# Wendison/FCL-taco2

Hardware: AMD Instinct MI355X
Metric: mel-frames/sec (FCL-taco2-S forward, batch=32, 80-mel) (higher is better)
Workload: dtype f32 via bf16x3-split MFMA operands, fp32 accumulate (max-abs 8e-6 on mel vs the reference; FCL_PRECISION=0 = exact fp32 MFMA)

## Files before the change

fcl-taco2_amd/csrc/capi.hip:

```cpp
#include <stdarg.h>
#include <stdlib.h>
#include <string.h>

#include <map>
#include <mutex>
#include <utility>
#include <vector>

#include "fcl_common.h"

namespace fcl {

static thread_local char g_err[512] = "";
static thread_local int g_gemm_mode = FCL_GEMM_F32;

void set_error(const char* fmt, ...) {
    va_list ap;
    va_start(ap, fmt);
    vsnprintf(g_err, sizeof(g_err), fmt, ap);
    va_end(ap);
}

int check_hip(hipError_t e, const char* what) {
    static const int sync_debug = getenv("FCL_SYNC_DEBUG") ? atoi(getenv("FCL_SYNC_DEBUG")) : 0;
// ... 505 lines not shown
        if (rc) return rc;
        GemmArgs f = {};
        f.term[0] = GemmTerm{io->att_c, w->wf_att, C, C, C, 0};
        if (planes) { f.term[0].Ap = io->att_c_p; f.term[0].Wp = w->wf_att_p; f.term[0].lda_p = f.term[0].ldw_p = ldc; }
        f.nterms = 1; f.M = N; f.N = O; f.Y = ws.F0; f.ldy = O;
        rc = launch_gemm(f, s);
        if (rc) return rc;
    }
    const float keep_scale = 1.0f / (1.0f - w->prenet_dropout);
    const int drop_mode = (w->prenet_dropout > 0.f) ? io->dropout_mode : FCL_DROP_NONE;
    {
        static const int tile_on = tunable("DEC_TILE", 0), tile_min = tunable("DEC_TILE_MIN_ROWS", 1024);
        if (tile_on && planes && w->stream && decoder_tile_shape_ok(w) && N >= tile_min && io->lmax <= 64 && !io->teacher_ys && !io->tap_prenet && !io->tap_lstm0 &&
            !io->tap_lstm1 && drop_mode != FCL_DROP_MASK && gemm_mode() != FCL_GEMM_BF16) {
            hipLaunchKernelGGL(zero_kernel, dim3(512), dim3(256), 0, s, ws.c0, (long long)((ws.c1 - ws.c0) + (size_t)N * U));
            FCL_HIP(hipGetLastError());
            return launch_decoder_tile(w, io, ws.G0, ws.F0, ws.c0, ws.c1, drop_mode, 0, nullptr, nullptr, s);
        }
    }
    const bool tile_ok = planes && w->stream && decoder_tile_shape_ok(w) && io->lmax <= 64 && !io->teacher_ys && !io->tap_prenet && !io->tap_lstm0 && !io->tap_lstm1 &&
                         drop_mode != FCL_DROP_MASK && gemm_mode() != FCL_GEMM_BF16;
    const int tail_from = (tile_ok && io->tail_from > 0 && io->tail_from < io->lmax) ? io->tail_from : 0;
    int cur = 0;
    for (int t = 0; t <= io->lmax; ++t) {
        const bool hand_over = tail_from > 0 && t == tail_from;
        const int n = (t < io->lmax && !hand_over) ? io->live_rows_host[t] : 0;
        const int n_prev = t > 0 ? io->live_rows_host[t - 1] : 0;
        const uint8_t* keep0 = drop_mode == FCL_DROP_MASK && t < io->lmax ? io->prenet_keep + ((size_t)(t * 2 + 0) * N) * P : nullptr;
        const uint8_t* keep1 = drop_mode == FCL_DROP_MASK && t < io->lmax ? io->prenet_keep + ((size_t)(t * 2 + 1) * N) * P : nullptr;
        const unsigned seed0 = io->seed * 2654435761u + (unsigned)(t * 2 + 0), seed1 = seed0 + 1;
        const float* teacher_in = (io->teacher_ys && t > 0) ? io->teacher_ys + (size_t)(t - 1) * O : nullptr;
        FeatPrenetArgs fp = {};
        fp.M_feat = n_prev; fp.M_pre = n; fp.U = U; fp.O = O; fp.P = P;
        fp.h1 = t > 0 ? ws.h1[cur] : nullptr; fp.wf_h = w->wf_h; fp.F0 = ws.F0;
        fp.before = io->before; fp.frame_off = io->frame_off; fp.t_prev = t - 1; fp.t_cur = t;
        fp.teacher_in = teacher_in; fp.teacher_ld = io->lmax * O;
        if (t < io->lmax && !hand_over) { fp.w0 = w->prenet_w0; fp.b0 = w->prenet_b0; fp.w1 = w->prenet_w1; fp.b1 = w->prenet_b1; }
        fp.wf_hi = w->wf_h_hi; fp.wf_lo = w->wf_h_lo; fp.w0_hi = w->prenet_w0_hi; fp.w0_lo = w->prenet_w0_lo;
        fp.w1_hi = w->prenet_w1_hi; fp.w1_lo = w->prenet_w1_lo;
        fp.wf_ff = w->wf_h_ff; fp.w0_ff = w->prenet_w0_ff; fp.w1_ff = w->prenet_w1_ff;
        fp.drop_mode = drop_mode; fp.keep0 = keep0; fp.keep1 = keep1; fp.keep_scale = keep_scale; fp.drop_p = w->prenet_dropout;
        fp.seed0 = seed0; fp.seed1 = seed1; fp.seed_dev = io->seed_dev; fp.pre_out = ws.pre_b; fp.tap_prenet = io->tap_prenet;
        fp.live = io->live_rows; fp.status = io->status; fp.out_act = w->out_act;
        if (planes) {
            fp.before_p = io->before_p;
            if (!small_step(n)) { fp.pre_out_p = ws.pre_p; fp.pre_out = nullptr; }
        }
        int rc = launch_feat_prenet(fp, s);
        if (rc) return rc;
        if (hand_over) return launch_decoder_tile(w, io, ws.G0, ws.F0, ws.c0, ws.c1, drop_mode, t, ws.h0[cur], ws.h1[cur], s);
        if (t == io->lmax) break;
        LstmStepArgs l0 = {};
        const bool big = planes && !small_step(n);
        const bool next_big = planes && t + 1 < io->lmax && !small_step(io->live_rows_host[t + 1]);
        l0.term[0] = GemmTerm{ws.pre_b, w->w0_pre, P, P, P, 0, w->w0_pre_hi, w->w0_pre_lo};
        l0.term[1] = GemmTerm{ws.h0[cur], w->w0_hh, U, U, U, 0, w->w0_hh_hi, w->w0_hh_lo};
        if (big) {
            l0.term[0].Ap = ws.pre_p; l0.term[0].Wp = w->w0_pre_p; l0.term[0].lda_p = l0.term[0].ldw_p = ldp;
            l0.term[1].Ap = ws.h0_p[cur]; l0.term[1].Wp = w->w0_hh_p; l0.term[1].lda_p = l0.term[1].ldw_p = ldu;
            l0.h_out_p = ws.h0_p[cur ^ 1]; l0.ld_hp = ldu;
        }
        l0.term[0].Wff = w->w0_pre_ff; l0.term[1].Wff = w->w0_hh_ff;
        l0.nterms = t == 0 ? 1 : 2; l0.M = n; l0.U = U; l0.G = ws.G0; l0.g_row_mul = 1; l0.g_row_add = 0;
        l0.m_dev = io->live_rows ? io->live_rows + t : nullptr;
        l0.rank1_w = w->w0_pos; l0.dur = io->dur; l0.step = t;
        l0.h_in = t == 0 ? nullptr : ws.h0[cur]; l0.h_out = ws.h0[cur ^ 1]; l0.c = ws.c0; l0.zoneout = w->zoneout_rate;
        if (io->tap_lstm0) { l0.out2 = io->tap_lstm0; l0.out2_row_base = io->frame_off; l0.out2_row_add = t; l0.ld2 = U; }
        rc = launch_lstm_step(l0, s);
        if (rc) return rc;
        LstmStepArgs l1 = {};
        l1.term[0] = GemmTerm{ws.h0[cur ^ 1], w->w1_ih, U, U, U, 0, w->w1_ih_hi, w->w1_ih_lo};
        l1.term[1] = GemmTerm{ws.h1[cur], w->w1_hh, U, U, U, 0, w->w1_hh_hi, w->w1_hh_lo};
        if (big) {
            l1.term[0].Ap = ws.h0_p[cur ^ 1]; l1.term[0].Wp = w->w1_ih_p; l1.term[0].lda_p = l1.term[0].ldw_p = ldu;
            l1.term[1].Ap = ws.h1_p[cur]; l1.term[1].Wp = w->w1_hh_p; l1.term[1].lda_p = l1.term[1].ldw_p = ldu;
            if (next_big) { l1.h_out_p = ws.h1_p[cur ^ 1]; l1.ld_hp = ldu; }
        }
        l1.term[0].Wff = w->w1_ih_ff; l1.term[1].Wff = w->w1_hh_ff;
        l1.nterms = t == 0 ? 1 : 2; l1.M = n; l1.U = U; l1.bias = w->b1; l1.step = t;
        l1.m_dev = l0.m_dev;
        l1.h_in = t == 0 ? nullptr : ws.h1[cur]; l1.h_out = ws.h1[cur ^ 1]; l1.c = ws.c1; l1.zoneout = w->zoneout_rate;
        if (io->tap_lstm1) { l1.out2 = io->tap_lstm1; l1.out2_row_base = io->frame_off; l1.out2_row_add = t; l1.ld2 = U; }
        rc = launch_lstm_step(l1, s);
        if (rc) return rc;
        cur ^= 1;
    }
    return 0;
}

}
```

fcl-taco2_amd/csrc/decoder_step.hip:

```cpp
#include "fcl_common.h"
#include "lstm_epilogue.h"

namespace fcl {


template <int NT>
__device__ __forceinline__ void rowtile_mma(const float* A_l, int lda_l, const float* const (&wrow)[NT], int K, int r16, int kq,
                                            f32x4 (&out)[NT], int rot = 0) {
    f32x4 acc0[NT], acc1[NT];
#pragma unroll
    for (int t = 0; t < NT; ++t) acc0[t] = acc1[t] = (f32x4){0.f, 0.f, 0.f, 0.f};
    const float* ap = A_l + r16 * lda_l + kq * 4;
    const float* wp[NT];
#pragma unroll
    for (int t = 0; t < NT; ++t) wp[t] = wrow[t] + kq * 4;
    const int nfull = K >> 6;
    f32x4 bn[NT][4];
    int cc = nfull > 0 ? rot % nfull : 0;
    if (nfull > 0) {
#pragma unroll
        for (int t = 0; t < NT; ++t)
#pragma unroll
            for (int i = 0; i < 4; ++i) bn[t][i] = *reinterpret_cast<const f32x4*>(wp[t] + (cc << 6) + i * 16);
    }
// ... 555 lines not shown

#ifdef FCL_FP_TS
constexpr int kFpTsWorkgroups = 1024;
__device__ long long g_fp_ts[kFpTsWorkgroups * 8 * 8];
struct FpStamps {
    long long t[8] = {0, 0, 0, 0, 0, 0, 0, 0};
    template <int I>
    __device__ __forceinline__ void at(bool drain = false) {
        __builtin_amdgcn_sched_barrier(0);
        if (drain) asm volatile("s_waitcnt vmcnt(0)" ::: "memory");
        asm volatile("s_memtime %0\n\ts_waitcnt lgkmcnt(0)" : "=s"(t[I])::"memory");
        __builtin_amdgcn_sched_barrier(0);
    }
    __device__ __forceinline__ void flush() {
        at<7>();
        if ((threadIdx.x & 63) == 0 && blockIdx.x < kFpTsWorkgroups) {
#pragma unroll
            for (int i = 0; i < 8; ++i) g_fp_ts[(blockIdx.x * 8 + (threadIdx.x >> 6)) * 8 + i] = t[i];
        }
    }
};
#define FP_STAMP(ts, i, ...) ts.at<i>(__VA_ARGS__)
#define FP_STAMP_FLUSH(ts) ts.flush()
#else
struct FpStamps {};
#define FP_STAMP(ts, i, ...)
#define FP_STAMP_FLUSH(ts)
#endif

template <class Ops, int DROP, int RT>
__global__ __launch_bounds__(512) void feat_prenet_split_kernel(const FeatPrenetArgs a) {
    typedef typename Ops::Tile Tile;
    constexpr int SU = 8, SO = 3, SP = 8, U = 256, OP = 96, P = 256;
    const int M_feat = a.M_feat, M_pre = a.M_pre;
    int Ms_feat, Ms_pre;
    if (!feat_prenet_rows(a, 16 * RT, Ms_feat, Ms_pre)) return;
    [[maybe_unused]] FpStamps ts;
    FP_STAMP(ts, 0);
    constexpr int ldU = U + Ops::PAD, ldO = OP + Ops::PAD, ldP = P + Ops::PAD, ROWS = 16 * RT;
    static_assert(ldU == ldP, "the layer-1 operand tile re-uses the h1 tile's LDS");
    auto* lds = Ops::dynamic_lds();
    const Tile A1 = Tile::carve(lds, ROWS * ldU);
    const Tile A2 = Tile::carve(lds, ROWS * ldO);
    const Tile A3 = A1;
    const int O = a.O;
    const int m0 = blockIdx.x * ROWS;
    const int lane = threadIdx.x & 63, wave = __builtin_amdgcn_readfirstlane(threadIdx.x >> 6);
    const int r16 = lane & 15, kq = lane >> 4;
    const int arow = lane & 15, cq = lane >> 4;
    const bool has_feat = a.h1 != nullptr, has_pre = a.w0 != nullptr && m0 < M_pre;
    const bool feat_wave = has_feat && wave * 16 < O;
    const size_t lane8 = (size_t)lane * 8;
    auto frag = [&](const typename Ops::W w, int tile, int ns) { return w.at((size_t)tile * ns * 512, lane8); };
    const int t0 = wave, t1 = wave + 8;
    const int c1 = wave * 2;

    constexpr int HV = RT * 2;
    f32x4 hreg[HV];
    if (has_feat) {
#pragma unroll
        for (int j = 0; j < HV; ++j) {
            const int i = threadIdx.x + j * 512, r = i >> 6, c = (i & 63) * 4;
            hreg[j] = *reinterpret_cast<const f32x4*>(a.h1 + (size_t)min(m0 + r, M_feat - 1) * U + c);
        }
    }
    asm volatile("s_barrier" ::: "memory");
    typename Ops::template Frag<1, SU> ff;
    typename Ops::template Frag<2, SO> f0;
    typename Ops::template Frag<2, SP> f1;
    const int fnc = wave * 16 + cq * 4;
    f32x4 f0v[RT];
    int fo[RT];
    if (feat_wave) {
        const typename Ops::W w[1] = {frag(Ops::wf(a), wave, SU)};
        ff.load(w);
    }
#pragma unroll
    for (int q = 0; q < RT; ++q) {
        f0v[q] = (f32x4){0.f, 0.f, 0.f, 0.f};
        fo[q] = 0;
        if (feat_wave && fnc < O) {
            const int mc = min(m0 + q * 16 + arow, M_feat - 1);
            f0v[q] = *reinterpret_cast<const f32x4*>(a.F0 + (size_t)mc * O + fnc);
            fo[q] = a.frame_off[mc];
        }
    }
    unsigned int seed0 = 0, seed1 = 0;
    const unsigned int thr16 = (unsigned int)(a.drop_p * 65536.0f);
    if (DROP == 2) {
        const unsigned int sbump = a.seed_dev ? *a.seed_dev * 0x9E3779B9u : 0u;
        seed0 = hash_u32(a.seed0 + sbump);
        seed1 = hash_u32(a.seed1 + sbump);
    }
    f32x4 pb0[2], pb1[2];
    unsigned int k0[RT][2], k1[RT][2];
#pragma unroll
    for (int tt = 0; tt < 2; ++tt) pb0[tt] = (f32x4){0.f, 0.f, 0.f, 0.f};
    if (has_feat) asm volatile("s_barrier" ::: "memory");
    if (has_pre) {
        const typename Ops::W w[2] = {frag(Ops::w0(a), t0, SO), frag(Ops::w0(a), t1, SO)};
        f0.load(w);
#pragma unroll
        for (int tt = 0; tt < 2; ++tt) {
            const int nc = (tt ? t1 : t0) * 16 + cq * 4;
            pb0[tt] = *reinterpret_cast<const f32x4*>(a.b0 + nc);
            if (DROP == 1) {
#pragma unroll
                for (int q = 0; q < RT; ++q) k0[q][tt] = *reinterpret_cast<const unsigned int*>(a.keep0 + (size_t)min(m0 + q * 16 + arow, M_pre - 1) * P + nc);
            }
        }
    }
    Ops::zero(A2, ROWS * ldO);
    if (has_feat) {
#pragma unroll
        for (int j = 0; j < HV; ++j) {
            const int i = threadIdx.x + j * 512, r = i >> 6, c = (i & 63) * 4;
// ... 2 lines not shown
    }
    FP_STAMP(ts, 1);
#pragma unroll
    for (int tt = 0; tt < 2; ++tt) pb1[tt] = (f32x4){0.f, 0.f, 0.f, 0.f};
    auto request_l1 = [&]() {
        if (has_pre) {
            typename Ops::W w[2];
#pragma unroll
            for (int tt = 0; tt < 2; ++tt) w[tt] = frag(Ops::w1(a), c1 + tt, SP);
            f1.load(w);
#pragma unroll
            for (int tt = 0; tt < 2; ++tt) {
                const int nc = (c1 + tt) * 16 + cq * 4;
                pb1[tt] = *reinterpret_cast<const f32x4*>(a.b1 + nc);
                if (DROP == 1) {
#pragma unroll
                    for (int q = 0; q < RT; ++q) k1[q][tt] = *reinterpret_cast<const unsigned int*>(a.keep1 + (size_t)min(m0 + q * 16 + arow, M_pre - 1) * P + nc);
                }
            }
        }
    };
    lds_barrier();
    FP_STAMP(ts, 2);
    if (feat_wave) {
#pragma unroll
        for (int q = 0; q < RT; ++q) {
            f32x4 accv[1];
            ff.mma_t(A1.at(q * 16 * ldU), ldU, r16, kq, accv);
            const int row = q * 16 + arow, m = m0 + row;
            if (fnc < O) {
                f32x4 v = (f32x4){0.f, 0.f, 0.f, 0.f};
                if (m < Ms_feat) {
                    v = accv[0] + f0v[q];
                    const long long fr = (long long)fo[q] + a.t_prev;
                    *reinterpret_cast<f32x4*>(a.before + (size_t)fr * O + fnc) = v;
                    if constexpr (Ops::kPlanes) {
                        if (a.before_p) {
                            uint2 h, l;
                            split4(v, h, l);
                            p32_store4(a.before_p, (O + 31) >> 5, fr, fnc, h, l);
                        }
                    }
                    if (a.out_act) {
#pragma unroll
                        for (int r = 0; r < 4; ++r) v[r] = act_apply(v[r], a.out_act);
                    }
                }
                Ops::store4(A2, row, ldO, fnc, v);
            }
        }
    }
    if (Ops::kPlanes && has_feat && a.before_p && (O & 31)) {
        const int padc = 32 - (O & 31);
        for (int i = threadIdx.x; i < ROWS * padc; i += 512) {
            const int m = m0 + i / padc;
            if (m < Ms_feat) store_p32(a.before_p, (O + 31) >> 5, a.frame_off[m] + a.t_prev, O + i % padc, 0.f);
        }
    }
    FP_STAMP(ts, 3);
    if (!has_pre) {
        FP_STAMP_FLUSH(ts);
        return;
    }
    request_l1();
    lds_barrier();
    if constexpr (Ops::kPlanes) {
        if (a.teacher_in) {
#pragma unroll
            for (int q = 0; q < RT; ++q) load_rowtile_split(A2.h + q * 16 * ldO, A2.l + q * 16 * ldO, ldO, a.teacher_in, a.teacher_ld, O, m0 + q * 16, M_pre);
            lds_barrier();
        }
    }
    FP_STAMP(ts, 4);
#pragma unroll
    for (int q = 0; q < RT; ++q) {
        f32x4 accv[2];
        f0.mma_t(A2.at(q * 16 * ldO), ldO, r16, kq, accv);
        const int row = q * 16 + arow, m = m0 + row;
#pragma unroll
// ... 14 lines not shown
        f32x4 accv[2];
        f1.mma_t(A3.at(q * 16 * ldP), ldP, r16, kq, accv);
        const int m = m0 + q * 16 + arow;
        if (m >= Ms_pre) continue;
#pragma unroll
        for (int tt = 0; tt < 2; ++tt) {
            const int nc = (c1 + tt) * 16 + cq * 4;
            f32x4 v = accv[tt] + pb1[tt];
#pragma unroll
            for (int r = 0; r < 4; ++r) v[r] = fmaxf(v[r], 0.f);
            v = drop4<DROP>(v, DROP == 1 ? k1[q][tt] : 0u, (unsigned int)m * (unsigned int)P + (unsigned int)nc, seed1, thr16, a.keep_scale);
            if (a.pre_out) *reinterpret_cast<f32x4*>(a.pre_out + (size_t)m * P + nc) = v;
            if constexpr (Ops::kPlanes) {
                if (a.pre_out_p) {
                    uint2 h, l;
                    split4(v, h, l);
                    p32_store4(a.pre_out_p, SP, m, nc, h, l);
                }
            }
            if (a.tap_prenet) *reinterpret_cast<f32x4*>(a.tap_prenet + (size_t)(a.frame_off[m] + a.t_cur) * P + nc) = v;
        }
    }
    FP_STAMP_FLUSH(ts);
}

__device__ __forceinline__ void glds16_unseen(const void* g, const void* l) {
    typedef const __attribute__((address_space(3))) void* lds_t;
    const unsigned dst = __builtin_amdgcn_readfirstlane((unsigned)(uintptr_t)(lds_t)l);
    unsigned keep;
    asm volatile("s_mov_b32 %0, m0\n\ts_mov_b32 m0, %2\n\ts_nop 0\n\tglobal_load_lds_dwordx4 %1, off\n\ts_mov_b32 m0, %0" : "=&s"(keep) : "v"(g), "s"(dst) : "memory");
}

template <int DROP, bool FEAT, bool PRE>
__device__ __forceinline__ void feat_prenet_walk(const FeatPrenetArgs& a, const int ntw, const int Ms_feat, const int Ms_pre) {
    typedef OpsX3 Ops;
    typedef Ops::Tile Tile;
    constexpr int SU = 8, SO = 3, SP = 8, U = 256, OP = 96, P = 256;
    constexpr int ldU = U + Ops::PAD, ldO = OP + Ops::PAD, ldP = P + Ops::PAD;
    constexpr int BUF = 2 * 16 * (ldU + ldO);
    static_assert(ldU == ldP, "the layer-1 operand tile re-uses the h1 tile's LDS");
    const int M_feat = a.M_feat, M_pre = a.M_pre;
    [[maybe_unused]] FpStamps ts;
    FP_STAMP(ts, 0);
    const int O = a.O;
    const int lane = threadIdx.x & 63, wave = __builtin_amdgcn_readfirstlane(threadIdx.x >> 6);
    const int r16 = lane & 15, kq = lane >> 4;
// ... 51 lines not shown
                const int i = threadIdx.x + j * 512, r = i >> 6, c = (i & 63) * 4;
                Ops::store4(A1.at(buf * BUF), r, ldU, c, hrow[j]);
            }
        }
    };

    if (feat_wave) {
        const Ops::W w = frag(Ops::wf(a), wave, SU);
#pragma unroll
        for (int st = 0; st < SU; ++st) {
            glds16_unseen(w.hi + st * 512, WF + st * 512);
            glds16_unseen(w.lo + st * 512, WF + (SU + st) * 512);
        }
    }
    request_rows(mbeg);
    asm volatile("s_barrier" ::: "memory");
    request_feat(mbeg);
    request_keep(k0, a.keep0, mbeg, t0, t1);
    request_keep(k1, a.keep1, mbeg, c1, c1 + 1);
    Ops::Frag<2, SO> f0;
    Ops::Frag<2, SP> f1;
    unsigned int seed0 = 0, seed1 = 0;
    const unsigned int thr16 = (unsigned int)(a.drop_p * 65536.0f);
    if (DROP == 2) {
        const unsigned int sbump = a.seed_dev ? *a.seed_dev * 0x9E3779B9u : 0u;
        seed0 = hash_u32(a.seed0 + sbump);
        seed1 = hash_u32(a.seed1 + sbump);
    }
    f32x4 bias = (f32x4){0.f, 0.f, 0.f, 0.f};
    const bool bias_thread = pre_any && threadIdx.x < 2 * (P / 4);
    if (pre_any) {
        if (bias_thread) bias = *reinterpret_cast<const f32x4*>((threadIdx.x < P / 4 ? a.b0 : a.b1 - P) + threadIdx.x * 4);
        const Ops::W w0[2] = {frag(Ops::w0(a), t0, SO), frag(Ops::w0(a), t1, SO)};
        f0.load(w0);
        const Ops::W w1[2] = {frag(Ops::w1(a), c1, SP), frag(Ops::w1(a), c1 + 1, SP)};
        f1.load(w1);
    }
    store_rows(0);
    if (bias_thread) *reinterpret_cast<f32x4*>(BL + threadIdx.x * 4) = bias;
    FP_STAMP(ts, 1);

    auto tile = [&](const int q) {
        const int buf = q & 1, m0 = mbeg + q * 16;
        const Tile T1 = A1.at(buf * BUF), T2 = A2.at(buf * BUF);
        const bool has_pre = pre_any && m0 < M_pre;
        lds_barrier();
        if (q == 0) FP_STAMP(ts, 2);
        if (feat_wave) {
            f32x4 acc = (f32x4){0.f, 0.f, 0.f, 0.f};
            const u16* ah = T1.h + r16 * ldU + kq * 8;
            const u16* al = T1.l + r16 * ldU + kq * 8;
            const u16* wf = WF + lane8;
#pragma unroll
            for (int st = 0; st < SU; ++st) {
                const s16x8 a_hi = *reinterpret_cast<const s16x8*>(ah + st * 32), a_lo = *reinterpret_cast<const s16x8*>(al + st * 32);
                const s16x8 w_hi = *reinterpret_cast<const s16x8*>(wf + st * 512), w_lo = *reinterpret_cast<const s16x8*>(wf + (SU + st) * 512);
                acc = __builtin_amdgcn_mfma_f32_16x16x32_bf16(w_hi, a_lo, acc, 0, 0, 0);
                acc = __builtin_amdgcn_mfma_f32_16x16x32_bf16(w_lo, a_hi, acc, 0, 0, 0);
                acc = __builtin_amdgcn_mfma_f32_16x16x32_bf16(w_hi, a_hi, acc, 0, 0, 0);
            }
            const int m = m0 + arow;
            if (fnc < O) {
                f32x4 v = (f32x4){0.f, 0.f, 0.f, 0.f};
                if (m < Ms_feat) {
                    v = acc + f0v;
                    const long long fr = (long long)fo + a.t_prev;
                    *reinterpret_cast<f32x4*>(a.before + (size_t)fr * O + fnc) = v;
                    if (a.before_p) {
                        uint2 h, l;
                        split4(v, h, l);
                        p32_store4(a.before_p, (O + 31) >> 5, fr, fnc, h, l);
                        if (pad_lane) p32_store4(a.before_p, (O + 31) >> 5, fr, padc, make_uint2(0u, 0u), make_uint2(0u, 0u));
                    }
                    if (a.out_act) {
#pragma unroll
                        for (int r = 0; r < 4; ++r) v[r] = act_apply(v[r], a.out_act);
                    }
                }
                Ops::store4(T2, arow, ldO, fnc, v);
            }
        }
        request_rows(m0 + 16);
        request_feat(m0 + 16);
        if (q == 0) FP_STAMP(ts, 3);
        f32x4 out1[2];
        if (has_pre) {
            lds_barrier();
            if (a.teacher_in) {
                load_rowtile_split(T2.h, T2.l, ldO, a.teacher_in, a.teacher_ld, O, m0, M_pre);
                lds_barrier();
            }
            if (q == 0) FP_STAMP(ts, 4);
            {
                f32x4 accv[2];
                f0.mma_t(T2, ldO, r16, kq, accv);
                const int m = m0 + arow;
#pragma unroll
                for (int tt = 0; tt < 2; ++tt) {
                    const int nc = (tt ? t1 : t0) * 16 + cq * 4;
                    f32x4 v = accv[tt] + *reinterpret_cast<const f32x4*>(BL + nc);
#pragma unroll
                    for (int r = 0; r < 4; ++r) v[r] = fmaxf(v[r], 0.f);
                    v = drop4<DROP>(v, DROP == 1 ? k0[tt] : 0u, (unsigned int)m * (unsigned int)P + (unsigned int)nc, seed0, thr16, a.keep_scale);
                    Ops::store4(T1, arow, ldP, nc, v);
                }
            }
            request_keep(k0, a.keep0, m0 + 16, t0, t1);
            lds_barrier();
            if (q == 0) {
                FP_STAMP(ts, 5);
                FP_STAMP(ts, 6, true);
            }
            f1.mma_t(T1, ldP, r16, kq, out1);
        }
        store_rows(buf ^ 1);
        asm volatile("" : "+v"(f0v), "+v"(fo), "+v"(k0[0]), "+v"(k0[1]));
        if (has_pre) {
            const int m = m0 + arow;
            if (m < Ms_pre) {
#pragma unroll
                for (int tt = 0; tt < 2; ++tt) {
                    const int nc = (c1 + tt) * 16 + cq * 4;
                    f32x4 v = out1[tt] + *reinterpret_cast<const f32x4*>(BL + P + nc);
#pragma unroll
                    for (int r = 0; r < 4; ++r) v[r] = fmaxf(v[r], 0.f);
                    v = drop4<DROP>(v, DROP == 1 ? k1[tt] : 0u, (unsigned int)m * (unsigned int)P + (unsigned int)nc, seed1, thr16, a.keep_scale);
                    if (a.pre_out) *reinterpret_cast<f32x4*>(a.pre_out + (size_t)m * P + nc) = v;
                    if (a.pre_out_p) {
                        uint2 h, l;
                        split4(v, h, l);
                        p32_store4(a.pre_out_p, SP, m, nc, h, l);
                    }
                    if (a.tap_prenet) *reinterpret_cast<f32x4*>(a.tap_prenet + (size_t)(a.frame_off[m] + a.t_cur) * P + nc) = v;
                }
            }
            request_keep(k1, a.keep1, m0 + 16, c1, c1 + 1);
        }
    };
    tile(0);
#pragma unroll 1
    for (int q = 1; q < nt; ++q) tile(q);
    FP_STAMP_FLUSH(ts);
}

template <int DROP>
__global__ __launch_bounds__(512) void feat_prenet_walk_kernel(const FeatPrenetArgs a, const int ntw) {
    int Ms_feat, Ms_pre;
    if (!feat_prenet_rows(a, 16 * ntw, Ms_feat, Ms_pre)) return;
    const bool pre = a.w0 != nullptr && (int)blockIdx.x * 16 * ntw < a.M_pre;
    if (a.h1 != nullptr) {
        if (pre) feat_prenet_walk<DROP, true, true>(a, ntw, Ms_feat, Ms_pre);
        else feat_prenet_walk<DROP, true, false>(a, ntw, Ms_feat, Ms_pre);
    } else if (pre) {
        feat_prenet_walk<DROP, false, true>(a, ntw, Ms_feat, Ms_pre);
    }
}

__device__ __forceinline__ void gates_to_cell(const LstmStepArgs& a, int g, int lane, const f32x4& acc, bool units_in_lane, int m, int u, bool valid, int Ms,
                                              const CellIn& ci) {
    __shared__ float g_l[4][16][17];
    const int lo = lane & 15, hi = lane >> 4;
#pragma unroll
    for (int i = 0; i < 4; ++i) {
        if (units_in_lane) g_l[g][lo][hi * 4 + i] = acc[i];
        else g_l[g][hi * 4 + i][lo] = acc[i];
    }
    __syncthreads();
    if (!valid || m >= Ms) return;
    const int row = threadIdx.x >> 4, uc = threadIdx.x & 15;
    const float pre[4] = {g_l[0][row][uc], g_l[1][row][uc], g_l[2][row][uc], g_l[3][row][uc]};
    cell_finish(a, m, u, pre, ci);
}

constexpr int kSmallStepsAtEntry = 4;

template <class Ops, int NT>
__device__ __forceinline__ f32x4 small_walk(const LstmStepArgs& a, typename Ops::Tile A, int ldk, int m0, int M, int g, int u0, int lane) {
// ... 193 lines not shown
        }
    }
    fprintf(stderr, "fp_ts %s rows %d workgroups %d: cycles since entry, mean (max):", form, rows, wgs);
    static const char* const name[8] = {"", "rows->LDS", "barrier0", "phase1", "barrier1", "phase2+barrier2", "all landed", "exit"};
    for (int i = 1; i < 8; ++i) fprintf(stderr, "  %s %.0f (%.0f)", name[i], cnt[i] ? sum[i] / cnt[i] : 0.0, mx[i]);
    fprintf(stderr, "\n");
    void* p = nullptr;
    if (hipGetSymbolAddress(&p, HIP_SYMBOL(g_fp_ts)) == hipSuccess) (void)hipMemset(p, 0, sizeof(h));
}
#else
static void print_fp_stamps(const char*, int, int) {}
#endif

static int launch_feat_prenet_walk(const FeatPrenetArgs& a, int rows, int ntw, hipStream_t s) {
    const size_t lds_w = sizeof(u16) * ((size_t)((a.O + 15) / 16) * 2 * 8 * 512 + 2 * 2 * 16 * ((256 + OpsX3::PAD) + (96 + OpsX3::PAD))) + 2 * 256 * sizeof(float);
    static const void* const fn[3] = {reinterpret_cast<const void*>(feat_prenet_walk_kernel<0>), reinterpret_cast<const void*>(feat_prenet_walk_kernel<1>),
                                      reinterpret_cast<const void*>(feat_prenet_walk_kernel<2>)};
    const int tiles = (rows + 15) / 16, wgs = (tiles + ntw - 1) / ntw;
    const int rc = launch_fp_drop(fn, a.drop_mode, dim3(wgs, 1), lds_w, a, s, ntw);
    if (!rc) print_fp_stamps("walk", rows, wgs);
    return rc;
}

template <class Ops, int RT>
static int launch_feat_prenet_split(const FeatPrenetArgs& a, int rows, hipStream_t s) {
    constexpr size_t lds_s = (size_t)Ops::LDS_BYTES * 16 * RT * ((256 + Ops::PAD) + (96 + Ops::PAD));
    static const void* const fn[3] = {reinterpret_cast<const void*>(feat_prenet_split_kernel<Ops, 0, RT>), reinterpret_cast<const void*>(feat_prenet_split_kernel<Ops, 1, RT>),
                                      reinterpret_cast<const void*>(feat_prenet_split_kernel<Ops, 2, RT>)};
    const int wgs = (rows + 16 * RT - 1) / (16 * RT);
    const int rc = launch_fp_drop(fn, a.drop_mode, dim3(wgs, 1), lds_s, a, s);
    if (!rc && Ops::kPlanes) print_fp_stamps(RT == 2 ? "split RT=2" : "split RT=1", rows, wgs);
    return rc;
}

int launch_feat_prenet(const FeatPrenetArgs& a, hipStream_t s) {
    const int rows = a.h1 ? a.M_feat : a.M_pre;
    if (rows <= 0) return 0;
    FCL_REQUIRE(!(a.U & 3) && !(a.O & 3) && !(a.P & 3), FCL_ERR_SHAPE, "feat_prenet: U/O/P must be multiples of 4");
    const size_t lds = sizeof(float) * 16 * ((size_t)(a.U + 4) + (a.O + 4) + (a.P + 4));
    FCL_REQUIRE(lds <= 160 * 1024, FCL_ERR_SHAPE, "feat_prenet: tile does not fit LDS (%zu B)", lds);
    double fl = 0;
    if (a.h1) fl += 2.0 * a.M_feat * a.O * a.U;
    if (a.w0) fl += 2.0 * a.M_pre * ((double)a.P * a.O + (double)a.P * a.P);
    const bool planes = a.wf_hi && a.wf_lo && a.w0_hi && a.w0_lo && a.w1_hi && a.w1_lo && !(a.U & 7) && !(a.O & 7) && !(a.P & 7);
    FCL_REQUIRE(planes || (!a.pre_out_p && !a.before_p), FCL_ERR_INVALID, "feat_prenet: P32 outputs need the bf16x3 weight planes");
    FCL_REQUIRE(!a.w0 || a.pre_out || a.pre_out_p, FCL_ERR_INVALID, "feat_prenet: no prenet output buffer");
    FCL_REQUIRE(!a.pre_out_p || !(a.P & 31), FCL_ERR_SHAPE, "feat_prenet: P32 prenet output needs P %% 32 == 0");
    if (planes) {
        const bool resident = a.U == 256 && a.O > 64 && a.O <= 96 && a.P == 256;
        static const int walk_tiles = tunable("FP_WALK_TILES", 2), walk_min = tunable("FP_WALK_MIN_TILES", 112);
        const bool walk = resident && walk_tiles > 0 && rows < 4096 && (rows + 15) / 16 >= walk_min;
        ProfScope ps(walk ? "feat_prenet_walk_kernel/bf16x3" : "feat_prenet_kernel/bf16x3", fl, rows, s);
        if (walk) {
            const int rc = launch_feat_prenet_walk(a, rows, walk_tiles, s);
            if (rc) return rc;
        } else if (resident) {
            const int rc = rows >= 4096 ? launch_feat_prenet_split<OpsX3, 2>(a, rows, s) : launch_feat_prenet_split<OpsX3, 1>(a, rows, s);
            if (rc) return rc;
        } else {
            const size_t lds3 = 2 * sizeof(unsigned short) * 16 * ((size_t)(a.U + 8) + (a.O + 8) + (a.P + 8));
            const int rc = ensure_dyn_lds(reinterpret_cast<const void*>(feat_prenet_x3_kernel), 160 * 1024);
            if (rc) return rc;
            hipLaunchKernelGGL(feat_prenet_x3_kernel, dim3((rows + 15) / 16), dim3(512), lds3, s, a);
        }
    } else if (a.wf_ff && a.w0_ff && a.w1_ff && a.U == 256 && a.P == 256 && a.O > 64 && a.O <= 96 && !a.teacher_in && !a.pre_out_p && !a.before_p &&
               (!a.w0 || a.pre_out)) {
        ProfScope ps("feat_prenet_split_kernel/f32", fl, rows, s);
        const int rc = launch_feat_prenet_split<OpsF32, 1>(a, rows, s);
        if (rc) return rc;
    } else {
        ProfScope ps("feat_prenet_kernel", fl, rows, s);
        const int rc = ensure_dyn_lds(reinterpret_cast<const void*>(feat_prenet_kernel), 160 * 1024);
        if (rc) return rc;
        hipLaunchKernelGGL(feat_prenet_kernel, dim3((rows + 15) / 16), dim3(512), lds, s, a);
    }
    return check_hip(hipGetLastError(), "feat_prenet launch");
// ... 4 lines not shown
```

fcl-taco2_amd/csrc/fcl_common.h:

```cpp
#pragma once
#include <hip/hip_runtime.h>
#include <stdint.h>
#include <stdio.h>

#include "../../include/fcl_hip.h"

namespace fcl {

void set_error(const char* fmt, ...);
int check_hip(hipError_t e, const char* what);

#define FCL_REQUIRE(cond, code, ...)            \
    do {                                        \
        if (!(cond)) {                          \
            ::fcl::set_error(__VA_ARGS__);      \
            return (code);                      \
        }                                       \
    } while (0)

#define FCL_HIP(expr)                                         \
    do {                                                      \
        int _rc = ::fcl::check_hip((expr), #expr);            \
        if (_rc != 0) return _rc;                             \
    } while (0)
// ... 88 lines not shown
    const float* h1;
    const float* wf_h;
    const float* F0;
    float* before;
    const int* frame_off;
    int t_prev, t_cur;
    const float* teacher_in;
    int teacher_ld;
    const float *w0, *b0, *w1, *b1;
    const unsigned short *wf_hi, *wf_lo, *w0_hi, *w0_lo, *w1_hi, *w1_lo;
    const float *wf_ff, *w0_ff, *w1_ff;
    int drop_mode;
    const uint8_t *keep0, *keep1;
    float keep_scale, drop_p;
    unsigned int seed0, seed1;
    const unsigned int* seed_dev;
    float* pre_out;
    float* tap_prenet;
    unsigned short* pre_out_p;
    unsigned short* before_p;
    const int* live;
    unsigned int* status;
    int out_act;
};

int row_maps_check(const fcl_row_maps_t* a, bool* fusable);
struct CellBwdArgs {
    const float *gates, *c_old, *c_new, *dh_out, *dh_out2, *dc_out;
    const uint8_t *zk_h, *zk_c;
    const int32_t* row_len;
    float *dgates, *dh_old, *dc_old;
    unsigned short* dgates_p;
    int ld_dh, ld_dho, ld_dh2, step, m, u;
    float zoneout;
};
int launch_lstm_cell_bwd(const CellBwdArgs& a, hipStream_t stream);
int launch_lstm_cell_bwd_pair(const CellBwdArgs& a0, const CellBwdArgs& a1, hipStream_t stream);
int launch_lstm_cell_bwd(const float* gates, const float* c_old, const float* c_new, const float* dh_out, int ld_dh, const float* dh_out2, int ld_dh2,
                         const float* dc_out, float zoneout, const uint8_t* zone_keep_h, const uint8_t* zone_keep_c, const int32_t* row_len, int step,
                         float* dgates, float* dh_old, int ld_dho, float* dc_old, uint16_t* dgates_p, int m, int u, hipStream_t stream);

__device__ __forceinline__ int live_rows_of(int m_host, const int* m_dev) { return m_dev ? min(m_host, *m_dev) : m_host; }

typedef float f32x4 __attribute__((ext_vector_type(4)));
typedef short s16x8 __attribute__((ext_vector_type(8)));
typedef unsigned short u16;
// ... 105 lines not shown
```

Baseline: 54.52 million.

## Add paired-tile feat/prenet kernel reading h1 planes directly, behind FP_PAIRS flag

Adds a new feat_prenet pair kernel that processes 32-row tiles, reusing each weight fragment across two row tiles, and reads the bf16 hi/lo planes of h1 straight into LDS instead of re-splitting fp32 h1. The decoder loop now passes h1 planes to the feat/prenet step. The split kernel is specialised on whether the prenet runs, the seed load is issued early and hashed after the barrier, and the before_p pad zeroing moves into the main store lanes. The pair path is off by default (FP_PAIRS=0), so by default only the split-kernel tweaks and the extra plane pointer take effect.

```diff
diff --git a/fcl-taco2_amd/csrc/capi.hip b/fcl-taco2_amd/csrc/capi.hip
--- a/fcl-taco2_amd/csrc/capi.hip
+++ b/fcl-taco2_amd/csrc/capi.hip
@@ -551,6 +551,7 @@
                          drop_mode != FCL_DROP_MASK && gemm_mode() != FCL_GEMM_BF16;
     const int tail_from = (tile_ok && io->tail_from > 0 && io->tail_from < io->lmax) ? io->tail_from : 0;
     int cur = 0;
+    bool h1_planes = false;
     for (int t = 0; t <= io->lmax; ++t) {
         const bool hand_over = tail_from > 0 && t == tail_from;
         const int n = (t < io->lmax && !hand_over) ? io->live_rows_host[t] : 0;
@@ -574,6 +575,7 @@
         if (planes) {
             fp.before_p = io->before_p;
             if (!small_step(n)) { fp.pre_out_p = ws.pre_p; fp.pre_out = nullptr; }
+            if (h1_planes) { fp.h1_p = ws.h1_p[cur]; fp.ld_h1p = ldu; }
         }
         int rc = launch_feat_prenet(fp, s);
         if (rc) return rc;
@@ -612,6 +614,7 @@
         if (io->tap_lstm1) { l1.out2 = io->tap_lstm1; l1.out2_row_base = io->frame_off; l1.out2_row_add = t; l1.ld2 = U; }
         rc = launch_lstm_step(l1, s);
         if (rc) return rc;
+        h1_planes = l1.h_out_p != nullptr;
         cur ^= 1;
     }
     return 0;
diff --git a/fcl-taco2_amd/csrc/decoder_step.hip b/fcl-taco2_amd/csrc/decoder_step.hip
--- a/fcl-taco2_amd/csrc/decoder_step.hip
+++ b/fcl-taco2_amd/csrc/decoder_step.hip
@@ -601,19 +601,39 @@
 };
 #define FP_STAMP(ts, i, ...) ts.at<i>(__VA_ARGS__)
 #define FP_STAMP_FLUSH(ts) ts.flush()
+#ifndef FCL_FP_TS_TILE
+#define FCL_FP_TS_TILE 0
+#endif
+#define FP_STAMP_ON(q, first) ((q) == FCL_FP_TS_TILE && (FCL_FP_TS_TILE == 0) == (first))
+#define FP_STAMP_IF(c, ts, i, ...) \
+    do {                           \
+        if (c) ts.at<i>(__VA_ARGS__); \
+    } while (0)
 #else
 struct FpStamps {};
 #define FP_STAMP(ts, i, ...)
+#define FP_STAMP_IF(c, ts, i, ...)
 #define FP_STAMP_FLUSH(ts)
 #endif
 
-template <class Ops, int DROP, int RT>
-__global__ __launch_bounds__(512) void feat_prenet_split_kernel(const FeatPrenetArgs a) {
+__device__ __forceinline__ unsigned int request_seed_word(const unsigned int* seed_dev) {
+    if (!seed_dev) return 0u;
+    int z = 0;
+    asm volatile("" : "+v"(z));
+    return seed_dev[z];
+}
+__device__ __forceinline__ void seeds_from_word(const FeatPrenetArgs& a, unsigned int word, unsigned int& seed0, unsigned int& seed1) {
+    __builtin_amdgcn_sched_barrier(0);
+    const unsigned int sbump = (unsigned int)__builtin_amdgcn_readfirstlane((int)word) * 0x9E3779B9u;
+    seed0 = hash_u32(a.seed0 + sbump);
+    seed1 = hash_u32(a.seed1 + sbump);
+}
+
+template <class Ops, int DROP, int RT, bool PRE>
+__device__ __forceinline__ void feat_prenet_split(const FeatPrenetArgs& a, const int Ms_feat, const int Ms_pre) {
     typedef typename Ops::Tile Tile;
     constexpr int SU = 8, SO = 3, SP = 8, U = 256, OP = 96, P = 256;
     const int M_feat = a.M_feat, M_pre = a.M_pre;
-    int Ms_feat, Ms_pre;
-    if (!feat_prenet_rows(a, 16 * RT, Ms_feat, Ms_pre)) return;
     [[maybe_unused]] FpStamps ts;
     FP_STAMP(ts, 0);
     constexpr int ldU = U + Ops::PAD, ldO = OP + Ops::PAD, ldP = P + Ops::PAD, ROWS = 16 * RT;
@@ -627,7 +647,8 @@
     const int lane = threadIdx.x & 63, wave = __builtin_amdgcn_readfirstlane(threadIdx.x >> 6);
     const int r16 = lane & 15, kq = lane >> 4;
     const int arow = lane & 15, cq = lane >> 4;
-    const bool has_feat = a.h1 != nullptr, has_pre = a.w0 != nullptr && m0 < M_pre;
+    const bool has_feat = a.h1 != nullptr;
+    constexpr bool has_pre = PRE;
     const bool feat_wave = has_feat && wave * 16 < O;
     const size_t lane8 = (size_t)lane * 8;
     auto frag = [&](const typename Ops::W w, int tile, int ns) { return w.at((size_t)tile * ns * 512, lane8); };
@@ -648,6 +669,8 @@
     typename Ops::template Frag<2, SO> f0;
     typename Ops::template Frag<2, SP> f1;
     const int fnc = wave * 16 + cq * 4;
+    const int padc = O + wave * 16 + cq * 4;
+    const bool pad_lane = wave < 2 && padc < ((O + 31) & ~31);
     f32x4 f0v[RT];
     int fo[RT];
     if (feat_wave) {
@@ -666,11 +689,7 @@
     }
     unsigned int seed0 = 0, seed1 = 0;
     const unsigned int thr16 = (unsigned int)(a.drop_p * 65536.0f);
-    if (DROP == 2) {
-        const unsigned int sbump = a.seed_dev ? *a.seed_dev * 0x9E3779B9u : 0u;
-        seed0 = hash_u32(a.seed0 + sbump);
-        seed1 = hash_u32(a.seed1 + sbump);
-    }
+    const unsigned int sword = DROP == 2 ? request_seed_word(a.seed_dev) : 0u;
     f32x4 pb0[2], pb1[2];
     unsigned int k0[RT][2], k1[RT][2];
 #pragma unroll
@@ -719,6 +738,7 @@
     };
     lds_barrier();
     FP_STAMP(ts, 2);
+    if (DROP == 2) seeds_from_word(a, sword, seed0, seed1);
     if (feat_wave) {
 #pragma unroll
         for (int q = 0; q < RT; ++q) {
@@ -729,13 +749,16 @@
                 f32x4 v = (f32x4){0.f, 0.f, 0.f, 0.f};
                 if (m < Ms_feat) {
                     v = accv[0] + f0v[q];
-                    const long long fr = (long long)fo[q] + a.t_prev;
+                    int fq = fo[q];
+                    asm volatile("" : "+v"(fq));
+                    const long long fr = (long long)fq + a.t_prev;
                     *reinterpret_cast<f32x4*>(a.before + (size_t)fr * O + fnc) = v;
                     if constexpr (Ops::kPlanes) {
                         if (a.before_p) {
                             uint2 h, l;
                             split4(v, h, l);
                             p32_store4(a.before_p, (O + 31) >> 5, fr, fnc, h, l);
+                            if (pad_lane) p32_store4(a.before_p, (O + 31) >> 5, fr, padc, make_uint2(0u, 0u), make_uint2(0u, 0u));
                         }
                     }
                     if (a.out_act) {
@@ -745,13 +768,6 @@
                 }
                 Ops::store4(A2, row, ldO, fnc, v);
             }
-        }
-    }
-    if (Ops::kPlanes && has_feat && a.before_p && (O & 31)) {
-        const int padc = 32 - (O & 31);
-        for (int i = threadIdx.x; i < ROWS * padc; i += 512) {
-            const int m = m0 + i / padc;
-            if (m < Ms_feat) store_p32(a.before_p, (O + 31) >> 5, a.frame_off[m] + a.t_prev, O + i % padc, 0.f);
         }
     }
     FP_STAMP(ts, 3);
@@ -812,6 +828,14 @@
         }
     }
     FP_STAMP_FLUSH(ts);
+}
+
+template <class Ops, int DROP, int RT>
+__global__ __launch_bounds__(512) void feat_prenet_split_kernel(const FeatPrenetArgs a) {
+    int Ms_feat, Ms_pre;
+    if (!feat_prenet_rows(a, 16 * RT, Ms_feat, Ms_pre)) return;
+    if (a.w0 != nullptr && (int)blockIdx.x * 16 * RT < a.M_pre) feat_prenet_split<Ops, DROP, RT, true>(a, Ms_feat, Ms_pre);
+    else feat_prenet_split<Ops, DROP, RT, false>(a, Ms_feat, Ms_pre);
 }
 
 __device__ __forceinline__ void glds16_unseen(const void* g, const void* l) {
@@ -909,11 +933,7 @@
     Ops::Frag<2, SP> f1;
     unsigned int seed0 = 0, seed1 = 0;
     const unsigned int thr16 = (unsigned int)(a.drop_p * 65536.0f);
-    if (DROP == 2) {
-        const unsigned int sbump = a.seed_dev ? *a.seed_dev * 0x9E3779B9u : 0u;
-        seed0 = hash_u32(a.seed0 + sbump);
-        seed1 = hash_u32(a.seed1 + sbump);
-    }
+    const unsigned int sword = DROP == 2 ? request_seed_word(a.seed_dev) : 0u;
     f32x4 bias = (f32x4){0.f, 0.f, 0.f, 0.f};
     const bool bias_thread = pre_any && threadIdx.x < 2 * (P / 4);
     if (pre_any) {
@@ -923,6 +943,7 @@
         const Ops::W w1[2] = {frag(Ops::w1(a), c1, SP), frag(Ops::w1(a), c1 + 1, SP)};
         f1.load(w1);
     }
+    if (DROP == 2) seeds_from_word(a, sword, seed0, seed1);
     store_rows(0);
     if (bias_thread) *reinterpret_cast<f32x4*>(BL + threadIdx.x * 4) = bias;
     FP_STAMP(ts, 1);
@@ -931,8 +952,9 @@
         const int buf = q & 1, m0 = mbeg + q * 16;
         const Tile T1 = A1.at(buf * BUF), T2 = A2.at(buf * BUF);
         const bool has_pre = pre_any && m0 < M_pre;
+        FP_STAMP_IF(FP_STAMP_ON(q, false), ts, 1);
         lds_barrier();
-        if (q == 0) FP_STAMP(ts, 2);
+        FP_STAMP_IF(q == FCL_FP_TS_TILE, ts, 2);
         if (feat_wave) {
             f32x4 acc = (f32x4){0.f, 0.f, 0.f, 0.f};
             const u16* ah = T1.h + r16 * ldU + kq * 8;
@@ -969,7 +991,7 @@
         }
         request_rows(m0 + 16);
         request_feat(m0 + 16);
-        if (q == 0) FP_STAMP(ts, 3);
+        FP_STAMP_IF(q == FCL_FP_TS_TILE, ts, 3);
         f32x4 out1[2];
         if (has_pre) {
             lds_barrier();
@@ -977,7 +999,7 @@
                 load_rowtile_split(T2.h, T2.l, ldO, a.teacher_in, a.teacher_ld, O, m0, M_pre);
                 lds_barrier();
             }
-            if (q == 0) FP_STAMP(ts, 4);
+            FP_STAMP_IF(q == FCL_FP_TS_TILE, ts, 4);
             {
                 f32x4 accv[2];
                 f0.mma_t(T2, ldO, r16, kq, accv);
@@ -994,14 +1016,13 @@
             }
             request_keep(k0, a.keep0, m0 + 16, t0, t1);
             lds_barrier();
-            if (q == 0) {
-                FP_STAMP(ts, 5);
-                FP_STAMP(ts, 6, true);
-            }
+            FP_STAMP_IF(q == FCL_FP_TS_TILE, ts, 5);
+            FP_STAMP_IF(FP_STAMP_ON(q, true), ts, 6, true);
             f1.mma_t(T1, ldP, r16, kq, out1);
         }
         store_rows(buf ^ 1);
         asm volatile("" : "+v"(f0v), "+v"(fo), "+v"(k0[0]), "+v"(k0[1]));
+        FP_STAMP_IF(FP_STAMP_ON(q, false), ts, 6);
         if (has_pre) {
             const int m = m0 + arow;
             if (m < Ms_pre) {
@@ -1040,6 +1061,290 @@
         else feat_prenet_walk<DROP, true, false>(a, ntw, Ms_feat, Ms_pre);
     } else if (pre) {
         feat_prenet_walk<DROP, false, true>(a, ntw, Ms_feat, Ms_pre);
+    }
+}
+
+template <int NT, int NS>
+__device__ __forceinline__ void pair_chain(const OpsX3::Frag<NT, NS>& f, OpsX3::Tile A, int ldk, int r16, int kq, f32x4 (&out)[2][NT]) {
+    const u16* ah = A.h + r16 * ldk + kq * 8;
+    const u16* al = A.l + r16 * ldk + kq * 8;
+#pragma unroll
+    for (int j = 0; j < 2; ++j)
+#pragma unroll
+        for (int t = 0; t < NT; ++t) out[j][t] = (f32x4){0.f, 0.f, 0.f, 0.f};
+#pragma unroll
+    for (int st = 0; st < NS; ++st) {
+        s16x8 a_hi[2], a_lo[2];
+#pragma unroll
+        for (int j = 0; j < 2; ++j) {
+            a_hi[j] = *reinterpret_cast<const s16x8*>(ah + j * 16 * ldk + st * 32);
+            a_lo[j] = *reinterpret_cast<const s16x8*>(al + j * 16 * ldk + st * 32);
+        }
+#pragma unroll
+        for (int t = 0; t < NT; ++t)
+#pragma unroll
+            for (int j = 0; j < 2; ++j) out[j][t] = __builtin_amdgcn_mfma_f32_16x16x32_bf16(f.hi[t][st], a_lo[j], out[j][t], 0, 0, 0);
+#pragma unroll
+        for (int t = 0; t < NT; ++t)
+#pragma unroll
+            for (int j = 0; j < 2; ++j) out[j][t] = __builtin_amdgcn_mfma_f32_16x16x32_bf16(f.lo[t][st], a_hi[j], out[j][t], 0, 0, 0);
+#pragma unroll
+        for (int t = 0; t < NT; ++t)
+#pragma unroll
+            for (int j = 0; j < 2; ++j) out[j][t] = __builtin_amdgcn_mfma_f32_16x16x32_bf16(f.hi[t][st], a_hi[j], out[j][t], 0, 0, 0);
+    }
+}
+
+constexpr int kFpPairRow = 2 * 256 + 16;
+constexpr int kFpPairBuf = 32 * kFpPairRow;
+
+template <int DROP, bool FEAT, bool PRE>
+__device__ __forceinline__ void feat_prenet_pairs(const FeatPrenetArgs& a, const int npw, const int Ms_feat, const int Ms_pre) {
+    typedef OpsX3 Ops;
+    typedef Ops::Tile Tile;
+    constexpr int SU = 8, SO = 3, SP = 8, OP = 96, P = 256;
+    constexpr int ldA = kFpPairRow, ldO = OP + Ops::PAD, HB = kFpPairBuf;
+    const int M_feat = a.M_feat, M_pre = a.M_pre;
+    [[maybe_unused]] FpStamps ts;
+    FP_STAMP(ts, 0);
+    const int O = a.O;
+    const int lane = threadIdx.x & 63, wave = __builtin_amdgcn_readfirstlane(threadIdx.x >> 6);
+    const int r16 = lane & 15, kq = lane >> 4;
+    const int arow = lane & 15, cq = lane >> 4;
+    constexpr bool has_feat = FEAT, pre_any = PRE;
+    const bool feat_wave = has_feat && wave * 16 < O;
+    const int mbeg = blockIdx.x * 32 * npw;
+    const int np = min(npw, ((has_feat ? Ms_feat : Ms_pre) - mbeg + 31) >> 5);
+    u16* lds = Ops::dynamic_lds();
+    u16* const WF = lds + wave * (2 * SU * 512);
+    lds += ((O + 15) >> 4) * (2 * SU * 512);
+    u16* const A1b = lds;
+    lds += 2 * HB;
+    const Tile T2 = Tile::carve(lds, 32 * ldO);
+    auto h1_tile = [&](int buf) { return Tile{A1b + buf * HB, A1b + buf * HB + 256}; };
+    auto bias_at = [&](int layer, int nc) { return reinterpret_cast<float*>(A1b + layer * HB + (nc >> 3) * ldA + 512) + (nc & 7); };
+    const size_t lane8 = (size_t)lane * 8;
+    auto frag = [&](const Ops::W w, int tile, int ns) { return w.at((size_t)tile * ns * 512, lane8); };
+    const int t0 = wave, t1 = wave + 8;
+    const int c1 = wave * 2;
+    const int fnc = wave * 16 + cq * 4;
+    const int padc = O + wave * 16 + cq * 4;
+    const bool pad_lane = wave < 2 && padc < ((O + 31) & ~31);
+    const unsigned hsrc = (unsigned)(((lane & 31) >> 2) * 64 + (lane >> 5) * 32 + (lane & 3) * 8);
+    const unsigned ldh = (unsigned)a.ld_h1p * 64u;
+
+    f32x4 f0v[2] = {(f32x4){0.f, 0.f, 0.f, 0.f}, (f32x4){0.f, 0.f, 0.f, 0.f}};
+    int fo[2] = {0, 0};
+    unsigned int k0[2][2] = {{0u, 0u}, {0u, 0u}}, k1[2][2] = {{0u, 0u}, {0u, 0u}};
+    auto request_rows = [&](int m0, int buf) {
+        if (has_feat) {
+#pragma unroll
+            for (int i = 0; i < 4; ++i) {
+                const int r = wave * 4 + i;
+                glds16_unseen(a.h1_p + ((unsigned)min(m0 + r, M_feat - 1) * ldh + hsrc), A1b + buf * HB + r * ldA);
+            }
+        }
+    };
+    auto request_fo = [&](int m0) {
+        if (has_feat) {
+#pragma unroll
+            for (int j = 0; j < 2; ++j) fo[j] = a.frame_off[(unsigned)min(m0 + j * 16 + arow, M_feat - 1)];
+        }
+    };
+    auto request_feat = [&](int m0) {
+        if (feat_wave && fnc < O) {
+#pragma unroll
+            for (int j = 0; j < 2; ++j) f0v[j] = *reinterpret_cast<const f32x4*>(a.F0 + (unsigned)(min(m0 + j * 16 + arow, M_feat - 1) * O + fnc));
+        }
+    };
+    auto request_keep = [&](unsigned int (&k)[2][2], const uint8_t* keep, int m0, int ca, int cb) {
+        if (DROP == 1 && pre_any && m0 < M_pre) {
+            int cqs = cq * 4;
+            asm volatile("" : "+v"(cqs));
+#pragma unroll
+            for (int j = 0; j < 2; ++j) {
+                const unsigned mk = (unsigned)(min(m0 + j * 16 + arow, M_pre - 1) * P);
+                k[j][0] = *reinterpret_cast<const unsigned int*>(keep + mk + ca * 16 + cqs);
+                k[j][1] = *reinterpret_cast<const unsigned int*>(keep + mk + cb * 16 + cqs);
+            }
+        }
+    };
+
+    if (feat_wave) {
+        const Ops::W w = frag(Ops::wf(a), wave, SU);
+#pragma unroll
+        for (int st = 0; st < SU; ++st) {
+            glds16_unseen(w.hi + st * 512, WF + st * 512);
+            glds16_unseen(w.lo + st * 512, WF + (SU + st) * 512);
+        }
+    }
+    request_rows(mbeg, 0);
+    request_fo(mbeg);
+    asm volatile("s_barrier" ::: "memory");
+    request_feat(mbeg);
+    request_keep(k0, a.keep0, mbeg, t0, t1);
+    request_keep(k1, a.keep1, mbeg, c1, c1 + 1);
+    Ops::Frag<2, SO> f0;
+    Ops::Frag<2, SP> f1;
+    unsigned int seed0 = 0, seed1 = 0;
+    const unsigned int thr16 = (unsigned int)(a.drop_p * 65536.0f);
+    const unsigned int sword = DROP == 2 ? request_seed_word(a.seed_dev) : 0u;
+    f32x4 bias = (f32x4){0.f, 0.f, 0.f, 0.f};
+    const bool bias_thread = pre_any && threadIdx.x < 2 * (P / 4);
+    if (pre_any) {
+        if (bias_thread) bias = *reinterpret_cast<const f32x4*>((threadIdx.x < P / 4 ? a.b0 : a.b1 - P) + threadIdx.x * 4);
+        const Ops::W w0[2] = {frag(Ops::w0(a), t0, SO), frag(Ops::w0(a), t1, SO)};
+        f0.load(w0);
+        const Ops::W w1[2] = {frag(Ops::w1(a), c1, SP), frag(Ops::w1(a), c1 + 1, SP)};
+        f1.load(w1);
+    }
+    if (DROP == 2) seeds_from_word(a, sword, seed0, seed1);
+    Ops::zero(T2, 32 * ldO);
+    if (bias_thread) *reinterpret_cast<f32x4*>(bias_at(threadIdx.x >> 6, (threadIdx.x & 63) * 4)) = bias;
+    if constexpr (FEAT) asm volatile("" : "+v"(fo[0]), "+v"(fo[1]));
+    FP_STAMP(ts, 1);
+
+    auto pair = [&](const int q) {
+        const int buf = q & 1, m0 = mbeg + q * 32;
+        const Tile T1 = h1_tile(buf);
+        const bool has_pre = pre_any && m0 < M_pre;
+        FP_STAMP_IF(FP_STAMP_ON(q, false), ts, 1);
+        lds_barrier();
+        FP_STAMP_IF(q == FCL_FP_TS_TILE, ts, 2);
+        if (feat_wave) {
+            f32x4 acc[2] = {(f32x4){0.f, 0.f, 0.f, 0.f}, (f32x4){0.f, 0.f, 0.f, 0.f}};
+            const u16* ah = T1.h + r16 * ldA + kq * 8;
+            const u16* al = T1.l + r16 * ldA + kq * 8;
+            const u16* wf = WF + lane8;
+#pragma unroll
+            for (int st = 0; st < SU; ++st) {
+                const s16x8 w_hi = *reinterpret_cast<const s16x8*>(wf + st * 512), w_lo = *reinterpret_cast<const s16x8*>(wf + (SU + st) * 512);
+                s16x8 a_hi[2], a_lo[2];
+#pragma unroll
+                for (int j = 0; j < 2; ++j) {
+                    a_hi[j] = *reinterpret_cast<const s16x8*>(ah + j * 16 * ldA + st * 32);
+                    a_lo[j] = *reinterpret_cast<const s16x8*>(al + j * 16 * ldA + st * 32);
+                }
+#pragma unroll
+                for (int j = 0; j < 2; ++j) acc[j] = __builtin_amdgcn_mfma_f32_16x16x32_bf16(w_hi, a_lo[j], acc[j], 0, 0, 0);
+#pragma unroll
+                for (int j = 0; j < 2; ++j) acc[j] = __builtin_amdgcn_mfma_f32_16x16x32_bf16(w_lo, a_hi[j], acc[j], 0, 0, 0);
+#pragma unroll
+                for (int j = 0; j < 2; ++j) acc[j] = __builtin_amdgcn_mfma_f32_16x16x32_bf16(w_hi, a_hi[j], acc[j], 0, 0, 0);
+            }
+            if (fnc < O) {
+                int fncs = fnc;
+                asm volatile("" : "+v"(fncs));
+#pragma unroll
+                for (int j = 0; j < 2; ++j) {
+                    const int m = m0 + j * 16 + arow;
+                    f32x4 v = (f32x4){0.f, 0.f, 0.f, 0.f};
+                    if (m < Ms_feat) {
+                        v = acc[j] + f0v[j];
+                        const long long fr = (long long)fo[j] + a.t_prev;
+                        *reinterpret_cast<f32x4*>(a.before + (size_t)fr * O + fncs) = v;
+                        if (a.before_p) {
+                            uint2 h, l;
+                            split4(v, h, l);
+                            p32_store4(a.before_p, (O + 31) >> 5, fr, fncs, h, l);
+                            if (pad_lane) p32_store4(a.before_p, (O + 31) >> 5, fr, O + fncs, make_uint2(0u, 0u), make_uint2(0u, 0u));
+                        }
+                        if (a.out_act) {
+#pragma unroll
+                            for (int r = 0; r < 4; ++r) v[r] = act_apply(v[r], a.out_act);
+                        }
+                    }
+                    Ops::store4(T2, j * 16 + arow, ldO, fnc, v);
+                }
+            }
+        }
+        request_rows(m0 + 32, buf ^ 1);
+        request_fo(m0 + 32);
+        request_feat(m0 + 32);
+        FP_STAMP_IF(q == FCL_FP_TS_TILE, ts, 3);
+        f32x4 out1[2];
+        if (has_pre) {
+            lds_barrier();
+            if (a.teacher_in) {
+#pragma unroll
+                for (int j = 0; j < 2; ++j) load_rowtile_split(T2.h + j * 16 * ldO, T2.l + j * 16 * ldO, ldO, a.teacher_in, a.teacher_ld, O, m0 + j * 16, M_pre);
+                lds_barrier();
+            }
+            FP_STAMP_IF(q == FCL_FP_TS_TILE, ts, 4);
+            {
+                f32x4 accv[2][2];
+                pair_chain(f0, T2, ldO, r16, kq, accv);
+#pragma unroll
+                for (int j = 0; j < 2; ++j) {
+                    const int m = m0 + j * 16 + arow;
+#pragma unroll
+                    for (int tt = 0; tt < 2; ++tt) {
+                        const int nc = (tt ? t1 : t0) * 16 + cq * 4;
+                        f32x4 v = accv[j][tt] + *reinterpret_cast<const f32x4*>(bias_at(0, nc));
+#pragma unroll
+                        for (int r = 0; r < 4; ++r) v[r] = fmaxf(v[r], 0.f);
+                        v = drop4<DROP>(v, DROP == 1 ? k0[j][tt] : 0u, (unsigned int)m * (unsigned int)P + (unsigned int)nc, seed0, thr16, a.keep_scale);
+                        Ops::store4(T1, j * 16 + arow, ldA, nc, v);
+                    }
+                }
+            }
+            request_keep(k0, a.keep0, m0 + 32, t0, t1);
+            lds_barrier();
+            FP_STAMP_IF(q == FCL_FP_TS_TILE, ts, 5);
+            FP_STAMP_IF(FP_STAMP_ON(q, true), ts, 6, true);
+            f1.mma_t(T1, ldA, r16, kq, out1);
+        }
+        asm volatile("s_waitcnt vmcnt(0)" ::: "memory");
+        if constexpr (FEAT) asm volatile("" : "+v"(f0v[0]), "+v"(f0v[1]), "+v"(fo[0]), "+v"(fo[1]));
+        if constexpr (DROP == 1) asm volatile("" : "+v"(k0[0][0]), "+v"(k0[0][1]), "+v"(k0[1][0]), "+v"(k0[1][1]));
+        FP_STAMP_IF(FP_STAMP_ON(q, false), ts, 6);
+        if (has_pre) {
+            int cqs = cq * 4;
+            asm volatile("" : "+v"(cqs));
+#pragma unroll
+            for (int j = 0; j < 2; ++j) {
+                const int m = m0 + j * 16 + arow;
+                if (j == 1) {
+                    __builtin_amdgcn_sched_barrier(0);
+                    f1.mma_t(T1.at(16 * ldA), ldA, r16, kq, out1);
+                }
+                if (m < Ms_pre) {
+#pragma unroll
+                    for (int tt = 0; tt < 2; ++tt) {
+                        const int nc = (c1 + tt) * 16 + cqs;
+                        f32x4 v = out1[tt] + *reinterpret_cast<const f32x4*>(bias_at(1, nc));
+#pragma unroll
+                        for (int r = 0; r < 4; ++r) v[r] = fmaxf(v[r], 0.f);
+                        v = drop4<DROP>(v, DROP == 1 ? k1[j][tt] : 0u, (unsigned int)m * (unsigned int)P + (unsigned int)nc, seed1, thr16, a.keep_scale);
+                        if (a.pre_out) *reinterpret_cast<f32x4*>(a.pre_out + (size_t)m * P + nc) = v;
+                        if (a.pre_out_p) {
+                            uint2 h, l;
+                            split4(v, h, l);
+                            p32_store4(a.pre_out_p, SP, m, nc, h, l);
+                        }
+                        if (a.tap_prenet) *reinterpret_cast<f32x4*>(a.tap_prenet + (size_t)(a.frame_off[m] + a.t_cur) * P + nc) = v;
+                    }
+                }
+            }
+            request_keep(k1, a.keep1, m0 + 32, c1, c1 + 1);
+        }
+    };
+    pair(0);
+#pragma unroll 1
+    for (int q = 1; q < np; ++q) pair(q);
+    FP_STAMP_FLUSH(ts);
+}
+
+template <int DROP>
+__global__ __launch_bounds__(512) void feat_prenet_pair_kernel(const FeatPrenetArgs a, const int npw) {
+    int Ms_feat, Ms_pre;
+    if (!feat_prenet_rows(a, 32 * npw, Ms_feat, Ms_pre)) return;
+    const bool pre = a.w0 != nullptr && (int)blockIdx.x * 32 * npw < a.M_pre;
+    if (a.h1 != nullptr) {
+        if (pre) feat_prenet_pairs<DROP, true, true>(a, npw, Ms_feat, Ms_pre);
+        else feat_prenet_pairs<DROP, true, false>(a, npw, Ms_feat, Ms_pre);
+    } else if (pre) {
+        feat_prenet_pairs<DROP, false, true>(a, npw, Ms_feat, Ms_pre);
     }
 }
 
@@ -1279,6 +1584,16 @@
     return rc;
 }
 
+static size_t fp_pair_lds(int O) { return sizeof(u16) * ((size_t)((O + 15) / 16) * 2 * 8 * 512 + 2 * kFpPairBuf + 2 * 32 * (96 + OpsX3::PAD)); }
+static int launch_feat_prenet_pairs(const FeatPrenetArgs& a, int rows, int npw, hipStream_t s) {
+    static const void* const fn[3] = {reinterpret_cast<const void*>(feat_prenet_pair_kernel<0>), reinterpret_cast<const void*>(feat_prenet_pair_kernel<1>),
+                                      reinterpret_cast<const void*>(feat_prenet_pair_kernel<2>)};
+    const int pairs = (rows + 31) / 32, wgs = (pairs + npw - 1) / npw;
+    const int rc = launch_fp_drop(fn, a.drop_mode, dim3(wgs, 1), fp_pair_lds(a.O), a, s, npw);
+    if (!rc) print_fp_stamps("pairs", rows, wgs);
+    return rc;
+}
+
 template <class Ops, int RT>
 static int launch_feat_prenet_split(const FeatPrenetArgs& a, int rows, hipStream_t s) {
     constexpr size_t lds_s = (size_t)Ops::LDS_BYTES * 16 * RT * ((256 + Ops::PAD) + (96 + Ops::PAD));
@@ -1306,9 +1621,15 @@
     if (planes) {
         const bool resident = a.U == 256 && a.O > 64 && a.O <= 96 && a.P == 256;
         static const int walk_tiles = tunable("FP_WALK_TILES", 2), walk_min = tunable("FP_WALK_MIN_TILES", 112);
+        static const int pairs_on = tunable("FP_PAIRS", 0), h1_planes_on = tunable("FP_H1_PLANES", 1);
         const bool walk = resident && walk_tiles > 0 && rows < 4096 && (rows + 15) / 16 >= walk_min;
+        const bool h1p_ok = h1_planes_on && a.h1_p && a.ld_h1p * 32 >= a.U && !(reinterpret_cast<uintptr_t>(a.h1_p) & 127u);
+        const bool pairs = walk && pairs_on && !(walk_tiles & 1) && (!a.h1 || h1p_ok) && fp_pair_lds(a.O) <= 160 * 1024;
         ProfScope ps(walk ? "feat_prenet_walk_kernel/bf16x3" : "feat_prenet_kernel/bf16x3", fl, rows, s);
-        if (walk) {
+        if (pairs) {
+            const int rc = launch_feat_prenet_pairs(a, rows, walk_tiles / 2, s);
+            if (rc) return rc;
+        } else if (walk) {
             const int rc = launch_feat_prenet_walk(a, rows, walk_tiles, s);
             if (rc) return rc;
         } else if (resident) {
diff --git a/fcl-taco2_amd/csrc/fcl_common.h b/fcl-taco2_amd/csrc/fcl_common.h
--- a/fcl-taco2_amd/csrc/fcl_common.h
+++ b/fcl-taco2_amd/csrc/fcl_common.h
@@ -134,6 +134,8 @@
     const int* live;
     unsigned int* status;
     int out_act;
+    const unsigned short* h1_p;
+    int ld_h1p;
 };
 
 int row_maps_check(const fcl_row_maps_t* a, bool* fusable);
```

Result: no change. 54.85 million, median of 6 (+0.6%).
